# 412428728/ksched

Hardware: AMD Instinct MI355X
Metric: MCMF solve latency (ms) + arcs/s at 100k tasks x 10k machines, 1/2/4/8 GPUs (higher is better)
Workload: dtype int64; 1 GPU; config3: Quincy-shaped cell graph T=100000 M=10000 R=250 J=1000 (n=121252, m=531250), step = full device re-solve + device task->PU extraction (Solve() -> TaskMapping), one graph per GPU; tasks=100000, machines=10000, racks=250, jobs=1000, seed=3, n=121252, m=531250, parallelism=independent graphs x1

## Files before the change

### ksched_amd/csrc/ks_engine.hip

```cpp
#include <hip/hip_runtime.h>

#include <algorithm>
#include <chrono>
#include <cstdio>
#include <cstdlib>
#include <cstring>
#include <vector>

#include "ks_engine_impl.h"

namespace ks {
namespace {

__device__ __forceinline__ void seg_of(const long long* nd, int x, int& b0, int& b1) {
    const unsigned long long w = (unsigned long long)nd[ni(x) + ND_SEG];
    b0 = (int)(unsigned)(w & 0xffffffffULL);
    b1 = (int)(unsigned)(w >> 32);
}

__device__ __forceinline__ long long atom_add_ret(long long* p, long long v) {
    return __hip_atomic_fetch_add(p, v, __ATOMIC_RELAXED, __HIP_MEMORY_SCOPE_AGENT);
}
__device__ __forceinline__ long long atom_exch(long long* p, long long v) {
    return __hip_atomic_exchange(p, v, __ATOMIC_RELAXED, __HIP_MEMORY_SCOPE_AGENT);
// ... 727 lines not shown
    const unsigned long long sg = (unsigned long long)__shfl(f.seg, src);
    b0 = (int)(unsigned)(sg & 0xffffffffULL);
    en = (int)(unsigned)(sg >> 32);
}

#define KS_AFTER_LOADS(c0, c1, ...) asm volatile("" : "+v"(c0), "+v"(c1) : __VA_ARGS__)

template <int C, bool CP>
__device__ __forceinline__ void sweep_win(const DG& g, const Front& N, int w, unsigned long long mask,
                                          const WinFlag& f, const long long* __restrict__ P,
                                          long long* __restrict__ PN, long long eps, Pend& pd, int& out, Cnt& c) {
    constexpr int G = class_lanes(C);
    constexpr int PER = 64 / G;
    constexpr int WS = win_slots(C);
    const int base = g.obeg[C] + (w - g.wbeg[C]) * WS;
    const int k = lane_id() / G;
    while (mask) {
        unsigned long long mm = mask;
        for (int j = 0; j < k; ++j) mm &= mm - 1;
        const int v = mm ? base + __ffsll((long long)mm) - 1 : -1;
        long long e = 0, pv = 0;
        int b0 = 0, en = 0;
        window_node(f, v, base, e, pv, b0, en);
        if (v < 0) e = 0;
        sweep_group<G, CP>(g, N, v, e, pv, b0, en, PN, P, eps, pd, out, c);
        for (int j = 0; j < PER; ++j) mask &= mask - 1;
    }
}


template <bool CP>
__global__ __launch_bounds__(BLK) void k_sweep(DG g, int pos, int seq) {
    if (pos == 0 && blockIdx.x == 0 && threadIdx.x == 0) g.ctl->t_sw0 = __builtin_amdgcn_s_memrealtime();
    if (blockIdx.x == 0)
        for (int h = threadIdx.x; h < g.nheavy; h += BLK) g.sf[(seq + 2) % 3].hub[h] = 0;
    int c_done, c_act;
    auto ctl_words = [&]() {
        c_done = g.ctl->bf_done;
        c_act = pos == 0 ? g.ctl->apply_act : g.ctl->sweep_act[pos - 1];
    };
    const Front F = g.sf[seq % 3], N = g.sf[(seq + 1) % 3];
    const long long eps = g.ctl->eps;
    const long long* P = (pos & 1) ? g.p1 : g.p0;
    long long* PN = (pos & 1) ? g.p0 : g.p1;
    Pend pd{-1, 0};
    Cnt c;
    int out = 0;
    if ((int)blockIdx.x < g.nhitems) {
        const HItem it = g.hitems[blockIdx.x];
        const int fl = F.hub[it.hid];
        const long long px = P[ni(it.node)];
        const long long E = atom_load(&g.excess[it.node]);
        ctl_words();
        KS_AFTER_LOADS(c_done, c_act, "v"(fl), "v"(px), "v"(E));
        if (c_done && c_act && fl) {
            hub_chunk<CP>(g, F, N, it, px, E, P, PN, eps, pd, out, c);
        }
    } else if ((int)blockIdx.x >= g.nhitems + g.sw_clsb) {
        const int i = (int)blockIdx.x - g.nhitems - g.sw_clsb;
        if (i < g.ncls_c) {
            const int x = g.obeg[CCLS] + i;
            const int fl = F.flag[x];
            const long long e = atom_load(&g.excess[x]);
            const long long px = P[ni(x)];
            const long long sw = g.p0[ni(x) + ND_SEG];
            ctl_words();
            KS_AFTER_LOADS(c_done, c_act, "v"(fl), "v"(e), "v"(px), "v"(sw));
            const int b0 = (int)(unsigned)((unsigned long long)sw & 0xffffffffULL);
            const int en = (int)(unsigned)((unsigned long long)sw >> 32);
            __shared__ long long s_e;
            __shared__ int s_go;
            if (threadIdx.x == 0) {
                s_e = e;
                s_go = c_done && c_act && fl;
            }
            __syncthreads();
            if (s_go) {
                node_discharge_blk<CP>(g, F, N, x, s_e, px, b0, en, PN, P, eps, pd, out, c);
            }
        }
    } else {
        const int tw = g.sw_clsb * WPB;
        const int w0 = wave_index_in_grid(g.nhitems);
        WinFlag wf[WPW];
        int any_raw = 0;
#pragma unroll
        for (int j = 0; j < WPW; ++j) {
            const int w = w0 + j * tw;
            wf[j] = w < g.wbeg[CCLS] ? window_load<1>(g, F.flag, w, P) : WinFlag{-1, 0, 0, 0, 0};
            any_raw |= wf[j].raw;
        }
        ctl_words();
        KS_AFTER_LOADS(c_done, c_act, "v"(any_raw));
        const bool go = c_done && c_act;
        unsigned long long mk[WPW];
#pragma unroll
        for (int j = 0; j < WPW; ++j) mk[j] = window_take(g, F.flag, w0 + j * tw, wf[j], go);
#pragma unroll
        for (int j = 0; j < WPW; ++j) {
            if (!mk[j]) continue;
            const int w = w0 + j * tw;
            switch (class_of_window(g, w)) {
                case 0: sweep_win<0, CP>(g, N, w, mk[j], wf[j], P, PN, eps, pd, out, c); break;
                case 1: sweep_win<1, CP>(g, N, w, mk[j], wf[j], P, PN, eps, pd, out, c); break;
                case 2: sweep_win<2, CP>(g, N, w, mk[j], wf[j], P, PN, eps, pd, out, c); break;
                case 3: sweep_win<3, CP>(g, N, w, mk[j], wf[j], P, PN, eps, pd, out, c); break;
                default: sweep_win<4, CP>(g, N, w, mk[j], wf[j], P, PN, eps, pd, out, c); break;
            }
        }
    }
    if (__any(out) && lane_id() == 0) g.ctl->sweep_act[pos] = 1;
    flush_counters(g, c);
}

constexpr int PK_NB = 24;
constexpr long long PK_NONE = (1LL << PK_NB) - 1;
constexpr long long PK_BIAS = 1LL << 37;
__device__ __forceinline__ long long pk(long long d, long long v) {
    d = d < 1 - PK_BIAS ? 1 - PK_BIAS : (d > PK_BIAS - 1 ? PK_BIAS - 1 : d);
    return ((d + PK_BIAS) << PK_NB) | v;
}
__device__ __forceinline__ long long pk_d(long long key) { return (key >> PK_NB) - PK_BIAS; }
template <int PR>
__device__ __forceinline__ long long dkey(long long raw) { return PR == 2 ? pk_d(raw) : raw; }
template <int PR>
__device__ __forceinline__ bool dless(long long a, long long b) { return PR == 2 ? (a >> PK_NB) < (b >> PK_NB) : a < b; }

template <int PR>
__device__ __forceinline__ long long arc_len(long long pu, long long ca, long long pv, long long eps) {
    long long len = floordiv(pu - ca - pv, eps) + 1;
    if (!PR) len = len < 0 ? 0 : (len > LEN_CAP ? LEN_CAP : len);
    return len;
}

template <int PR>
__device__ __forceinline__ bool offer(const DG& g, const Front& nf, int u, long long cand, long long du,
                                      long long B, long long* hub_min, int& out) {
    if (cand >= B) return false;
    if (u >= g.hub_base) {
        const int h = u - g.hub_base;
        if (h < HUB_LDS) {
            __hip_atomic_fetch_min(&hub_min[h], cand, __ATOMIC_RELAXED, __HIP_MEMORY_SCOPE_WORKGROUP);
        } else if (dless<PR>(cand, atom_min_ret(&g.dist[ni(u)], cand))) {
            nf.hub[h] = 1;
            out = 1;
        }
        return false;
    }
    if (!dless<PR>(cand, du)) return false;
    atom_min(&g.dist[ni(u)], cand);
    return true;
}

template <int PR, bool CP>
__device__ __forceinline__ void expand_leaf(const DG& g, const Front& nf, int u, long long du, long long pu,
                                            int b0, int b1, long long eps, long long B, long long* hub_min, int& out,
                                            long long& lscan) {
    lscan += b1 - b0;
    unsigned live = 0;
    int hd[8];
    long long cb[8];
#pragma unroll
    for (int k = 0; k < 8; ++k) {
        hd[k] = 0;
        cb[k] = 0;
        if (b0 + k < b1) {
            const Pos q = PL<CP>::ld_nr(g, b0 + k);
            hd[k] = q.head;
            cb[k] = q.cost;
            if (q.ucap - q.rcap > 0) live |= 1u << k;
        }
    }
    for (int b = b1 - b0 > 8 ? b0 + 8 : b1; b < b1; ++b) {
        const Pos q = PL<CP>::ld_nr(g, b);
        if (q.ucap - q.rcap > 0) {
            const int u2 = q.head;
            long long cand = du + arc_len<PR>(g.p0[ni(u2)], q.cost, pu, eps);
            if (PR == 2) cand = pk(cand, b);
            if (offer<PR>(g, nf, u2, cand, u2 < g.hub_base ? g.dist[ni(u2)] : INF64, B, hub_min, out)) {
                nf.flag[u2] = 1;
                out = 1;
            }
        }
    }
    while (live) {
        const int k = __builtin_ctz(live);
        live &= live - 1;
        int u2 = 0;
        long long c2 = 0;
#pragma unroll
        for (int j = 0; j < 8; ++j)
            if (j == k) {
                u2 = hd[j];
                c2 = cb[j];
            }
        const long long pu2 = g.p0[ni(u2)];
        const long long du2 = u2 < g.hub_base ? g.dist[ni(u2)] : INF64;
        long long cand = du + arc_len<PR>(pu2, c2, pu, eps);
        if (PR == 2) cand = pk(cand, b0 + k);
        if (offer<PR>(g, nf, u2, cand, du2, B, hub_min, out)) {
            nf.flag[u2] = 1;
            out = 1;
        }
    }
}

template <int PR, bool CP>
__device__ __forceinline__ void relax_in(const DG& g, const Front& nf, int v, int a, long long dv, long long pv,
                                         long long eps, long long B, long long* hub_min, int& out, long long& lscan) {
    const Pos q = PL<CP>::ld_nr(g, a);
    const long long rin = q.ucap - q.rcap;
    const int u = rin > 0 ? q.head : 0;
    const long long ca = q.cost;
    const long long pu = g.p0[ni(u)];
    const long long du = u < g.hub_base ? g.dist[ni(u)] : INF64;
    const bool leaf = g.expand && u < g.obeg[2];
    int b0 = 0, b1 = 0;
    if (leaf) seg_of(g.p0, u, b0, b1);
    if (rin <= 0) return;
    const long long cand = dv + arc_len<PR>(pu, ca, pv, eps);
    if (!offer<PR>(g, nf, u, PR == 2 ? pk(cand, a) : cand, du, B, hub_min, out)) return;
    if (leaf) {
        expand_leaf<PR, CP>(g, nf, u, cand, pu, b0, b1, eps, B, hub_min, out, lscan);
    } else {
        nf.flag[u] = 1;
        out = 1;
    }
}

template <int G, int PR, bool CP>
__device__ __forceinline__ void bf_group_pre(const DG& g, const Front& nf, int v, long long dv, long long pv, int b0,
                                             int en, long long eps, long long B, long long* hub_min, int& out, long long& scans, long long& lscan) {
    const int lig = lane_id() & (G - 1);
    const bool act = v >= 0 && (PR || dv < INF64);
    if (!act) en = b0;
    const int iters = G < 64 ? 1 : (en - b0 + 63) / 64;
    for (int it = 0; it < iters; ++it) {
        const int a = b0 + it * G + lig;
        if (a < en) {
            relax_in<PR, CP>(g, nf, v, a, dkey<PR>(dv), pv, eps, B, hub_min, out, lscan);
            scans++;
        }
    }
}

template <int C, int PR, bool CP>
__device__ __forceinline__ void bf_win(const DG& g, const Front& N, int w, unsigned long long mask, const WinFlag& f,
                                       long long eps, long long B, long long* hub_min, int& out, long long& scans, long long& lscan) {
    constexpr int G = class_lanes(C);
    constexpr int PER = 64 / G;
    constexpr int WS = win_slots(C);
    const int base = g.obeg[C] + (w - g.wbeg[C]) * WS;
    const int k = lane_id() / G;
    while (mask) {
        unsigned long long mm = mask;
        for (int j = 0; j < k; ++j) mm &= mm - 1;
        const int v = mm ? base + __ffsll((long long)mm) - 1 : -1;
        long long d = INF64, pv = 0;
        int b0 = 0, en = 0;
        window_node(f, v, base, d, pv, b0, en);
        if (v < 0) d = INF64;
        bf_group_pre<G, PR, CP>(g, N, v, d, pv, b0, en, eps, B, hub_min, out, scans, lscan);
        for (int j = 0; j < PER; ++j) mask &= mask - 1;
    }
}

template <int PR, bool CP>
__device__ __forceinline__ void bf_chunk(const DG& g, const Front& N, const CItem& ci, long long eps,
                                         long long B, long long* hub_min, int& out, long long& scans, long long& lscan) {
    const long long dv = atom_load(&g.dist[ni(ci.node)]);
    if (!PR && dv >= INF64) return;
    const int a = ci.begin + lane_id();
    if (a < ci.end) {
        relax_in<PR, CP>(g, N, ci.node, a, dkey<PR>(dv), g.p0[ni(ci.node)], eps, B, hub_min, out, lscan);
        scans++;
    }
}

template <int G, int PR, bool CP>
__device__ __forceinline__ void bf_group(const DG& g, const Front& nf, int v, long long eps, long long B, long long* hub_min,
                                         int& out, long long& scans, long long& lscan) {
    const int lig = lane_id() & (G - 1);
    long long dv = INF64;
    if (v >= 0) dv = atom_load(&g.dist[ni(v)]);
    const bool act = v >= 0 && (PR || dv < INF64);
    long long pv = 0;
    int b0 = 0, en = 0;
    if (act) {
        pv = g.p0[ni(v)];
        seg_of(g.p0, v, b0, en);
    }
    const int iters = G < 64 ? 1 : (en - b0 + 63) / 64;
    for (int it = 0; it < iters; ++it) {
        const int a = b0 + it * G + lig;
        if (a < en) {
            relax_in<PR, CP>(g, nf, v, a, dkey<PR>(dv), pv, eps, B, hub_min, out, lscan);
            scans++;
        }
    }
}

template <int PR, bool CP>
__global__ __launch_bounds__(BLK) void k_bf_round(DG g, int seq, int dense_arg) {
    const unsigned long long t_entry = PR == 2 ? __builtin_amdgcn_s_memrealtime() : 0;
    const int dense = dense_arg >= 0 ? dense_arg : (seq == g.ctl->bf_seq0 ? 1 : 0);
    __shared__ long long hub_min[HUB_LDS];
    if (blockIdx.x == 0) {
        for (int h = threadIdx.x; h < g.nheavy; h += BLK) g.bf[(seq + 2) % 3].hub[h] = 0;
        if (threadIdx.x == 0) g.ctl->bfa[(seq + 2) % 3] = 0;
    }
    const Front F = g.bf[seq % 3], N = g.bf[(seq + 1) % 3];
    if (threadIdx.x < HUB_LDS) hub_min[threadIdx.x] = INF64;
    __syncthreads();
    int done = 0, any = 0;
    auto ctl_words = [&]() {
        done = g.ctl->bf_done;
        any = g.ctl->bfa[seq % 3];
    };
    const long long eps = g.ctl->eps;
    const long long B = (!PR && g.bound) ? atom_load(&g.ctl->bf_bound) : INF64;
    int out = 0;
    long long scans = 0, lscan = 0;
    const int nhb = g.nhitems * HSPLIT;
    if ((int)blockIdx.x < nhb) {
        const HItem it = g.hitems[blockIdx.x / HSPLIT];
        const int sub = (int)blockIdx.x % HSPLIT;
        const int fl = F.hub[it.hid];
        const long long dv = atom_load(&g.dist[ni(it.node)]);
        const long long pv = g.p0[ni(it.node)];
        ctl_words();
        KS_AFTER_LOADS(done, any, "v"(fl), "v"(dv), "v"(pv));
        if (!done && (dense || any) && (dense || fl)) {
            if (PR || dv < INF64) {
#pragma unroll
                for (int k = 0; k < BF_PER_T; ++k) {
                    const int a = it.begin + sub * (CHUNK / HSPLIT) + threadIdx.x * BF_PER_T + k;
                    if (a < it.end) {
                        relax_in<PR, CP>(g, N, it.node, a, dkey<PR>(dv), pv, eps, B, hub_min, out, lscan);
                        scans++;
                    }
                }
            }
        }
    } else if (dense) {
        const int w = wave_index_in_grid(nhb);
        ctl_words();
        if (done) {
        } else if (w < g.wbeg[CCLS]) {
            const Scan sc{F.flag, 1};
#define KS_BF_CALL(C) bf_group<G_, PR, CP>(g, N, v, eps, B, hub_min, out, scans, lscan)
            KS_BY_CLASS(w, sc, KS_BF_CALL)
#undef KS_BF_CALL
        } else if (w - g.wbeg[CCLS] < g.ncitems) {
            bf_chunk<PR, CP>(g, N, g.citems[w - g.wbeg[CCLS]], eps, B, hub_min, out, scans, lscan);
        }
    } else {
        const int tw = ((int)gridDim.x - nhb) * WPB;
        const int w0 = wave_index_in_grid(nhb);
        WinFlag wf[WPW];
        int any_raw = 0;
#pragma unroll
        for (int j = 0; j < WPW; ++j) {
            wf[j] = window_load<2>(g, F.flag, w0 + j * tw);
            any_raw |= wf[j].raw;
        }
        ctl_words();
        KS_AFTER_LOADS(done, any, "v"(any_raw));
        const bool go = !done && any;
        unsigned long long mk[WPW];
#pragma unroll
        for (int j = 0; j < WPW; ++j) {
            const int w = w0 + j * tw;
            mk[j] = window_take(g, F.flag, w, wf[j], go);
            if (go && w >= g.wbeg[CCLS] && w - g.wbeg[CCLS] < g.ncitems && lane_id() == 0) {
                const CItem ci = g.citems[w - g.wbeg[CCLS]];
                if (ci.lead) g.bf[(seq + 2) % 3].flag[ci.node] = 0;
            }
        }
#pragma unroll
        for (int j = 0; j < WPW; ++j) {
            if (!mk[j]) continue;
            const int w = w0 + j * tw;
            if (w >= g.wbeg[CCLS]) {
                bf_chunk<PR, CP>(g, N, g.citems[w - g.wbeg[CCLS]], eps, B, hub_min, out, scans, lscan);
                continue;
            }
            switch (class_of_window(g, w)) {
                case 0: bf_win<0, PR, CP>(g, N, w, mk[j], wf[j], eps, B, hub_min, out, scans, lscan); break;
                case 1: bf_win<1, PR, CP>(g, N, w, mk[j], wf[j], eps, B, hub_min, out, scans, lscan); break;
                case 2: bf_win<2, PR, CP>(g, N, w, mk[j], wf[j], eps, B, hub_min, out, scans, lscan); break;
                case 3: bf_win<3, PR, CP>(g, N, w, mk[j], wf[j], eps, B, hub_min, out, scans, lscan); break;
                default: bf_win<4, PR, CP>(g, N, w, mk[j], wf[j], eps, B, hub_min, out, scans, lscan); break;
            }
        }
    }
    __syncthreads();
    if (threadIdx.x < HUB_LDS && (int)threadIdx.x < g.nheavy) {
        const long long val = hub_min[threadIdx.x];
        if (val < INF64) {
            long long* dx = &g.dist[ni(g.hub_base + threadIdx.x)];
            if (dless<PR>(val, atom_load(dx)) && dless<PR>(val, atom_min_ret(dx, val))) {
                N.hub[threadIdx.x] = 1;
                out = 1;
            }
        }
    }
    if (__any(out) && lane_id() == 0) g.ctl->bfa[(seq + 1) % 3] = 1;
    if (blockIdx.x == 0 && threadIdx.x == 0) {
        if (PR == 2 && g.ctl->t_srch) {
            g.ctl->srch_ticks += t_entry - g.ctl->t_srch;
            g.ctl->t_srch = 0;
        }
        if (!done && (dense || any)) {
            atomicAdd(g.ctr + C_BFROUND, 1ULL);
            g.ctl->bf_count += 1;
        } else if (!done) {
            g.ctl->bf_done = 1;
        }
    }
    if (!PR && g.bound && blockIdx.x == 0 && threadIdx.x < WAVE && !done && (dense || any)) {
        const int nb = g.ctl->n_bx;
        if (nb > 0 && nb <= BX_CAP) {
            long long d = 0;
            if ((int)threadIdx.x < nb) d = atom_load(&g.dist[ni(g.bx[threadIdx.x])]);
            d = wave_max(d);
            if (threadIdx.x == 0 && d < INF64)
                __hip_atomic_fetch_min(&g.ctl->bf_bound, d, __ATOMIC_RELAXED, __HIP_MEMORY_SCOPE_AGENT);
        }
    }
    scans = wave_sum(scans);
    lscan = wave_sum(lscan);
    if (lane_id() == 0 && (scans | lscan)) {
        const int sh = ((blockIdx.x * WPB) + (threadIdx.x >> 6)) & (CTR_SHARDS - 1);
        if (scans) atomicAdd(g.ctr + sh * NCTR + C_GUSCAN, (unsigned long long)scans);
        if (lscan) atomicAdd(g.ctr + sh * NCTR + C_GULEAF, (unsigned long long)lscan);
    }
}

__device__ __forceinline__ void clear_fronts(const DG& g, const Front* fs) {
    for (long long i = blockIdx.x * (long long)BLK + threadIdx.x; i < g.hub_base; i += (long long)gridDim.x * BLK) {
        fs[0].flag[i] = 0;
        fs[1].flag[i] = 0;
        fs[2].flag[i] = 0;
    }
    if (blockIdx.x == 0)
        for (int h = threadIdx.x; h < g.nheavy; h += BLK) fs[0].hub[h] = fs[1].hub[h] = fs[2].hub[h] = 0;
}

__device__ __forceinline__ void bx_append(const DG& g, bool on, int v) {
    const unsigned long long m = __ballot(on);
    if (!m) return;
    int base = 0;
    if (lane_id() == 0) base = atomicAdd(&g.ctl->n_bx, (int)__popcll(m));
    base = __shfl(base, 0);
    if (on) {
        const int idx = base + (int)__popcll(m & ((1ULL << lane_id()) - 1));
        if (idx < BX_CAP) g.bx[idx] = v;
    }
}

__global__ void k_gu_init(DG g, int seq0, int list) {
    if (g.ctl->gu_pending) return;
    clear_fronts(g, g.bf);
    const Front F0 = g.bf[seq0 % 3];
    if (blockIdx.x == 0 && threadIdx.x == 0) {
        __hip_atomic_store(&g.ctl->bf_bound, INF64, __ATOMIC_RELAXED, __HIP_MEMORY_SCOPE_AGENT);
        g.ctl->gu_B = INF64;
        g.ctl->bf_done = 0;
        g.ctl->gu_L = 0;
        g.ctl->gu_X = -1;
        g.ctl->bf_r0 = g.ctl->bf_count;
        g.ctl->bf_seq0 = seq0;
        g.ctl->n_exc = 0;
        g.ctl->u_exc = 0;
        g.ctl->aug_reached = 0;
        g.ctl->aug_short = 0;
        for (int k = 0; k < 3; ++k) g.ctl->bfa[k] = k == seq0 % 3 ? 1 : 0;
    }
    for (long long v0 = blockIdx.x * (long long)BLK; v0 < g.hub_base; v0 += (long long)gridDim.x * BLK) {
        const long long v = v0 + threadIdx.x;
        long long e = 0;
        if (v < g.hub_base) {
            e = atom_load(&g.excess[v]);
            g.dist[ni(v)] = e < 0 ? 0 : INF64;
            if (e < 0) F0.flag[v] = 1;
        }
        if (list) bx_append(g, e > 0, (int)v);
    }
    if (blockIdx.x == 0)
        for (int h0 = 0; h0 < g.nheavy; h0 += BLK) {
            const int h = h0 + threadIdx.x;
            long long e = 0;
            if (h < g.nheavy) {
                drain_inbox(g, h);
                e = atom_load(&g.excess[g.hub_base + h]);
                g.dist[ni(g.hub_base + h)] = e < 0 ? 0 : INF64;
                if (e < 0) F0.hub[h] = 1;
            }
            if (list) bx_append(g, e > 0, g.hub_base + h);
        }
}

__global__ void k_pr_init(DG g, int seq0, int from_p) {
    clear_fronts(g, g.bf);
    if (blockIdx.x == 0 && threadIdx.x == 0) {
        g.ctl->bf_done = 0;
        g.ctl->bf_seq0 = seq0;
        for (int k = 0; k < 3; ++k) g.ctl->bfa[k] = 0;
    }
    for (long long v = blockIdx.x * (long long)BLK + threadIdx.x; v < g.n; v += (long long)gridDim.x * BLK)
        g.dist[ni(v)] = from_p == 2 ? ((PK_BIAS << PK_NB) | PK_NONE) : from_p ? g.p0[ni(v)] : 0;
}

__global__ void k_cycle_end(DG g, Ctl* host, int fwd) {
    static_assert(sizeof(Ctl) % 4 == 0, "Ctl is copied as words");
    const unsigned long long t = __builtin_amdgcn_s_memrealtime();
    if (threadIdx.x == 0) {
        if (!fwd) g.ctl->gu_pending = g.ctl->bf_done ? 0 : 1;
        g.ctl->t_end = t;
    }
    __syncthreads();
    const int* src = reinterpret_cast<const int*>(g.ctl);
    int* dst = reinterpret_cast<int*>(host);
    for (int i = threadIdx.x; i < (int)(sizeof(Ctl) / 4); i += blockDim.x)
        __hip_atomic_store(&dst[i], src[i], __ATOMIC_RELAXED, __HIP_MEMORY_SCOPE_SYSTEM);
    __syncthreads();
    if (threadIdx.x == 0) {
        if (!fwd) {
            g.ctl->n_exc = 0;
            g.ctl->u_exc = 0;
        }
        g.ctl->fs_moved_cyc = 0;
    }
    __threadfence_system();
}

constexpr int SET_FWD = 1;
constexpr int SET_CYC = 2;
__global__ void k_set_eps(DG g, long long eps, int flags) {
    g.ctl->eps = eps;
    if (flags & SET_FWD) {
        g.ctl->fs_pending = 0;
        g.ctl->fs_cnt[0] = g.ctl->fs_cnt[1] = g.ctl->fs_cnt[2] = 0;
        g.ctl->fs_completed = 0;
    }
    if (flags & SET_CYC) {
        g.ctl->cyc_done = 0;
        g.ctl->cyc_rej = 0;
    }
// ... 1214 lines not shown
        int nsearch, cap, used;
        int nb;
        unsigned long long srch_seen;
    } fin{};

    SolveRun(EngineImpl& s_, ks_result& res_, std::string& err_, bool warm)
        : s(s_), res(res_), err(err_), o(s_.opts), st(s_.stream), fb(s_.fb_active),
          use_warm((warm && s_.has_prev) || s_.fb_active) {}

    double wall_s() const {
        return std::chrono::duration<double>(std::chrono::steady_clock::now() - t_host0).count();
    }

    int run() {
        int rc = prepare();
        if (rc || nn == 0) return rc;
        plan();
        if ((rc = warm_start())) return rc;
        rc = s.cell_layout ? cell_solve() : phase_loop();
        if (rc || retry != RETRY_NONE) return rc;
        if (cycle_log)
            std::fprintf(stderr, "solve phases %d updates %llu (forward %llu) early phase ends %llu\n", phases,
                         (unsigned long long)gus, (unsigned long long)fwd_updates, (unsigned long long)early_exits);
        if (status == KS_E_INFEASIBLE && !s.cell_layout)
            err = "infeasible: some supply cannot reach a demand node (code " + std::to_string(s.h_ctl->infeasible) +
                  ", phase " + std::to_string(phases) + ", eps " + std::to_string(eps) + ", updates " +
                  std::to_string(gus) + ", sweeps " + std::to_string(sweep_launches) + ")";
        KS_CHECK(hipEventRecord(s.ev[5], st));
        if (status == KS_OK && (rc = certify())) return rc;
        return report();
    }

    int prepare() {
        s.solved = false;
        {
            const bool cells_now = want_cells(s);
            if (cells_now != s.cell_layout) {
                s.cell_layout = cells_now;
                s.csr_valid = false;
            }
        }
        res.warm_started = use_warm ? 1 : 0;
        res.rebuilt = s.csr_valid ? 0 : 1;
        res.recoveries = 0;
        res.cell_fallbacks = 0;
        res.cycles_cancelled = 0;
        res.fb_resets = 0;
        res.cycles_rejected = 0;
        KS_CHECK(hipEventRecord(s.ev[0], st));
        KS_CHECK(hipMemsetAsync(s.ctr.p, 0, CTR_SHARDS * NCTR * sizeof(unsigned long long), st));
        KS_CHECK(hipMemsetAsync(s.ctl.p, 0, sizeof(Ctl), st));
        std::memset(s.h_ctl, 0, sizeof(Ctl));
        if (!s.csr_valid) {
            if (int rc = rebuild()) return rc;
        } else if (!use_warm) {
            if (int rc = cold_reset(s, err)) return rc;
        }
        hi = s.hi();
        nn = s.nn;
        m2 = s.m2cap;
        mult = s.mult;
        ncells = (int)s.h_cells.size();
        res.n_nodes = s.nslots;
        res.n_arcs = s.h_sctl->live;
        if (nn == 0) {
            res.total_cost = 0;
            res.flow_value = 0;
            s.solved = true;
            s.has_prev = true;
            return KS_OK;
        }
        if (hi)
            hipLaunchKernelGGL(k_max_cost, dim3(grid_for(hi, 512)), dim3(BLK), 0, st, hi,
                               (const unsigned char*)s.a_alive.p, (const long long*)s.a_cost.p, &s.ctl.p->gu_L);
        const bool want_cp = !s.cell_layout && s.opts.compact_pos >= 0 && m2 > 0;
        if (want_cp) {
            KS_CHECK(s.cpos.ensure(m2));
            KS_CHECK(s.crev.ensure(m2));
            hipLaunchKernelGGL(k_pack_pos, dim3(grid_for(m2, 4096)), dim3(BLK), 0, st, (long long)m2,
                               (const Pos*)s.pos.p, s.cpos.p, s.crev.p, &s.ctl.p->cp_bad);
        }
        KS_CHECK(read_ctl());
        maxc = s.h_ctl->gu_L;
        cpv = want_cp && !s.h_ctl->cp_bad;
        cp_dirty = false;
        res.compact = cpv ? 1 : 0;
        KS_CHECK(hipMemsetAsync(&s.ctl.p->gu_L, 0, sizeof(long long), st));
        if (maxc > 0 && (double)maxc * (double)mult * 8.0 * (double)mult > 4.0e18) {
            err = "cost range too large for int64 scaled prices";
            return KS_E_RANGE;
        }
        KS_CHECK(hipEventRecord(s.ev[1], st));
        return KS_OK;
    }

    int rebuild() {
        const int64_t ncap_prev = s.ncap;
        const long long mult_prev = s.mult;
        const bool carry = use_warm && s.nn > 0;
        const int hi0 = s.hi();
        if (carry) {
            KS_CHECK(s.saved_flows.ensure(std::max(hi0, 1)));
            KS_CHECK(s.p_slot.ensure(std::max<int64_t>(ncap_prev, 1)));
            if (hi0)
                hipLaunchKernelGGL(k_save_flows, dim3(grid_for(hi0)), dim3(BLK), 0, st, hi0,
                                   (const unsigned char*)s.a_alive.p, (const int*)s.fwd.p, (const Pos*)s.pos.p,
                                   s.saved_flows.p);
            hipLaunchKernelGGL(k_save_prices, dim3(grid_for(ncap_prev)), dim3(BLK), 0, st, (int)ncap_prev,
                               (const int*)s.perm.p, (const long long*)s.nd.p, s.p_slot.p);
            if (fb && !s.fb_cells.empty()) {
                std::vector<long long> rng;
                const size_t kc = s.cell_off.size() >= 2 ? s.cell_off.size() - 1 : 1;
                for (int c : s.fb_cells) {
                    rng.push_back(kc > 1 ? s.cell_off[c] : 0);
                    rng.push_back(kc > 1 ? s.cell_off[c + 1] : ncap_prev);
                }
                KS_CHECK(s.fb_rng.ensure(rng.size()));
                KS_CHECK(hipMemcpyAsync(s.fb_rng.p, rng.data(), rng.size() * sizeof(long long), hipMemcpyHostToDevice,
                                        st));
                const int n = (int)std::max<int64_t>(hi0, ncap_prev);
                KS_CHECK(s.fb_cnt.ensure(1));
                KS_CHECK(hipMemsetAsync(s.fb_cnt.p, 0, sizeof(unsigned long long), st));
                hipLaunchKernelGGL(k_fb_reset, dim3(grid_for(std::max(n, 1))), dim3(BLK), 0, st, hi0, (int)ncap_prev,
                                   (int)(rng.size() / 2), (const long long*)s.fb_rng.p, (const int*)s.a_src.p,
                                   (const unsigned char*)s.a_alive.p, s.saved_flows.p, s.p_slot.p, s.fb_cnt.p);
                unsigned long long nres = 0;
                KS_CHECK(hipMemcpyAsync(&nres, s.fb_cnt.p, sizeof(nres), hipMemcpyDeviceToHost, st));
                KS_CHECK(hipStreamSynchronize(st));
                res.fb_resets = nres;
            }
        }
        int rc = build(s, err);
        if (rc) return rc;
        rc = cold_reset(s, err);
        if (rc) return rc;
        if (carry) {
            if (hi0)
                hipLaunchKernelGGL(k_restore_flows, dim3(grid_for(hi0)), dim3(BLK), 0, st, hi0,
                                   (const unsigned char*)s.a_alive.p, (const long long*)s.saved_flows.p,
                                   (const long long*)s.a_low.p, (const long long*)s.a_cap.p, (const int*)s.fwd.p,
                                   (const int*)s.a_src.p, (const int*)s.a_dst.p, (const int*)s.perm.p, s.pos.p,
                                   s.excess.p);
            hipLaunchKernelGGL(k_restore_prices, dim3(grid_for(s.ncap)), dim3(BLK), 0, st, (int)s.ncap,
                               (int)ncap_prev, mult_prev, s.mult, (const long long*)s.p_slot.p, (const int*)s.perm.p,
                               s.nd.p, (s.nd.p + 2));
        }
        return KS_OK;
    }

    void plan() {
        g = s.dg();
        g.cp = cpv ? s.cpos.p : nullptr;
        g.crev = cpv ? s.crev.p : nullptr;
        g.expand = o.two_hop < 0 ? 0 : 1;
        g.bound = o.bf_bound < 0 ? 0 : 1;
        g.fs_wide = std::max(2048, nn / 4);
        g.aug_k = o.tail_nodes > 0 ? std::min(AUG_KMAX, (int)o.tail_nodes) : 64;
        fgrid = s.window_grid();
        dgrid = s.dense_grid();
        sgrid = s.sparse_grid();
        wgrid = s.sweep_grid();
        ngrid = grid_for(nn, 2048);
        fsgrid = s.nhitems * HSPLIT + FS_LIST_BLOCKS;
        vgrid = grid_for(hi, 2048);
        use_fwd = o.fwd_nodes >= 0 && s.m2cap < FS_NONE;
        fwd_k = o.fwd_nodes > 0 ? (int)o.fwd_nodes : (nn < 32768 ? 32 : 64);
        use_pr = o.price_refine != 0;
        use_prc = use_pr && o.price_refine == 1 && !s.cell_layout && s.m2cap < PK_NONE;
        alpha = o.alpha >= 2 ? o.alpha : (!s.cell_layout && nn < 32768 && use_prc) ? 32 : 8;
        gi_base = o.gu_interval > 0 ? o.gu_interval : 24;
        gi_base = std::max(2, std::min(MAXB, gi_base)) & ~1;
        pr_cap = o.pr_rounds > 0 ? o.pr_rounds : 160;
        cycle_log = o.log_cycles != 0;
        nhit = s.nhitems;
        use_aug = o.walk_slack >= 0;
        aug_slack = o.walk_slack > 0 ? o.walk_slack : 4;
        walk_passes = o.walk_passes > 0 ? std::min(8, (int)o.walk_passes) : 1;
        kb_margin = o.bf_margin > 0 ? o.bf_margin : 6;
        kb_min = 8;
        prc_cap = (o.fault_inject & 32) ? 32 : 4096;
        cyc_lg = (o.fault_inject & 128) ? 5 : CYC_LOG;
        gi_tail = o.tail_sweeps > 0 ? std::max(2, std::min(MAXB, (int)o.tail_sweeps)) & ~1 : 4;
        phase_exit = o.phase_exit < 0 ? 0 : (o.phase_exit > 0 ? o.phase_exit : 256);
        phase_frac = o.phase_frac > 0 ? o.phase_frac : 128;
        eps = std::max<long long>(1, maxc * mult);
        {
            const long long D = o.final_div < 0 ? 0
                                : o.final_div > 0 ? o.final_div
                                : (s.cell_layout || nn < 32768) ? 20 : (use_prc ? 24 : 48);
            if (D > 0 && use_pr && maxc > 0) {
                long long e = std::max<long long>(1, (mult - 1) / D);
                if (s.cell_layout && (alpha & (alpha - 1)) == 0)
                    while (e & (e - 1)) e &= e - 1;
                const long long lo = std::max<long long>(1, eps / ((long long)alpha * alpha));
                while (e < lo && e <= (1LL << 58) / alpha) e *= alpha;
                eps = e * alpha;
                pr_div = D;
            }
        }
        eps_start = eps;
    }

    int warm_start() {
        if (!use_warm || fb) return KS_OK;
        if (o.warm_shift >= 0)
            hipLaunchKernelGGL(k_price_shift, dim3(grid_for(s.ncap, 2048)), dim3(BLK), 0, st, (int)s.ncap,
                               (const unsigned long long*)s.n_cshift.p, (const int*)s.perm.p, mult, s.nd.p);
        hipLaunchKernelGGL(k_fresh_prices, dim3(grid_for(s.ncap, 2048)), dim3(BLK), 0, st, (int)s.ncap,
                           (const unsigned char*)s.n_fresh.p, (const int*)s.perm.p, g);
        if (m2) hipLaunchKernelGGL(k_max_viol, dim3(grid_for(m2, 2048)), dim3(BLK), 0, st, g, (long long)m2);
        KS_CHECK(read_ctl());
        const long long viol = s.h_ctl->gu_L;
        constexpr long long kWarmUnits = 8;
        long long e0 = std::max<long long>(1, std::min<long long>({viol, kWarmUnits * mult, eps}));
        if (s.cell_layout && (alpha & (alpha - 1)) == 0)
            while (e0 & (e0 - 1)) e0 += e0 & -e0;
        warm_thr = e0;
        eps = e0 * alpha;
        eps_start = eps;
        KS_CHECK(hipMemsetAsync(&s.ctl.p->gu_L, 0, sizeof(long long), st));
        if (cycle_log) {
            std::vector<long long> h((size_t)4 * nn);
            KS_CHECK(hipMemcpyAsync(h.data(), s.nd.p, h.size() * sizeof(long long), hipMemcpyDeviceToHost, st));
            KS_CHECK(hipStreamSynchronize(st));
            long long lo = INF64, hi2 = -INF64;
            for (int v = 0; v < nn; ++v) {
                lo = std::min(lo, h[(size_t)4 * v]);
                hi2 = std::max(hi2, h[(size_t)4 * v]);
            }
            std::fprintf(stderr, "warm start: largest violation %.3f units, first phase at %.3f units, price span %.1f units\n",
                         (double)viol / mult, (double)e0 / mult, (double)(hi2 - lo) / mult);
        }
        return KS_OK;
    }

    hipError_t read_ctl() {
        hipError_t e = hipMemcpyAsync(s.h_ctl, s.ctl.p, sizeof(Ctl), hipMemcpyDeviceToHost, st);
        if (e != hipSuccess) return e;
        return hipStreamSynchronize(st);
    }
    hipError_t set_eps(long long e, int flags = 0) {
        hipLaunchKernelGGL(k_set_eps, dim3(1), dim3(1), 0, st, g, e, flags);
        return hipGetLastError();
    }
    void bf_round(int mode, bool dense) {
        const int grid = dense ? dgrid : sgrid;
        if (mode == 2) launch_bf_round<2>(cpv, grid, st, g, bseq, dense ? 1 : 0);
        else if (mode) launch_bf_round<1>(cpv, grid, st, g, bseq, dense ? 1 : 0);
        else launch_bf_round<0>(cpv, grid, st, g, bseq, dense ? 1 : 0);
        ++bseq;
        ++bf_launches;
    }
    void bf_rounds(int mode, int k, bool first_dense) {
        for (int r = 0; r < k; ++r) bf_round(mode, first_dense && r == 0);
    }
    void sync_pos() {
        if (!cp_dirty) return;
        hipLaunchKernelGGL(k_unpack_pos, dim3(grid_for(m2, 4096)), dim3(BLK), 0, st, (long long)m2,
                           (const CPos*)s.cpos.p, s.pos.p);
        cp_dirty = false;
    }
    int relaxations(unsigned long long* since) {
        std::vector<unsigned long long> hctr((size_t)CTR_SHARDS * NCTR);
        KS_CHECK(hipMemcpy(hctr.data(), s.ctr.p, hctr.size() * sizeof(unsigned long long), hipMemcpyDeviceToHost));
        unsigned long long gsc = 0;
        for (int i = 0; i < CTR_SHARDS; ++i) gsc += hctr[(size_t)i * NCTR + C_GUSCAN];
        *since = gsc - gu_prev;
        gu_prev = gsc;
        return KS_OK;
    }

    bool is_last(long long e) const { return e / alpha < 1 || e <= 1 || (use_pr && e * pr_div < mult); }

    int phase_loop() {
        do {
            eps = std::max<long long>(1, eps / alpha);
            ++phases;
            long long sat_thr = phases == 1 && use_warm && !fb
                                    ? warm_thr
                                    : ((pr_failed || fb || (use_warm && o.warm_start >= 2)) ? eps : 0LL);
            pr_failed = false;
            const bool last_phase = is_last(eps);
            const long long eps_next = std::max<long long>(1, eps / alpha);
            const bool before_last = !last_phase && !prc_tried && is_last(eps_next);
            const bool prc_now = use_prc && before_last;
            const long long eps_next2 = std::max<long long>(1, eps_next / alpha);
            const bool before_last2 = !last_phase && !before_last && is_last(eps_next2);
            const int walk_sl = (eps > 1 || (o.fault_inject & 1)) ? aug_slack : 1;
            int prc_early = 0;
            const bool may_early = use_prc && !prc_tried && before_last2 && !use_warm && !fb && eps <= 2 * mult;
            const int rc = run_phase(eps, sat_thr, !last_phase && !prc_now, walk_sl, may_early ? &prc_early : nullptr);
            if (rc == KS_E_INFEASIBLE) {
                status = rc;
                break;
            }
            if (rc) return rc;
            if (prc_now || prc_early) {
                prc_tried = true;
                int used = 0;
                const int pr = finish(&used, prc_early ? std::min(prc_cap, 1024) : prc_cap);
                if (pr < 0) return pr;
                if (pr == 1) {
                    eps = 1;
                    break;
                }
                pr_failed = true;
                continue;
// ... 689 lines not shown
```

Baseline: 15.53 million arcs/s.

## Drain newly improved mid-class nodes in-block via LDS queue during Bellman-Ford round

Adds a per-block shared-memory queue in the Bellman-Ford relaxation kernel. Nodes in a middle class range whose distance improves are queued, and the block drains them right away by scanning their arcs with 32-lane groups, instead of flagging them for the next global round. The drain skips entries whose distance has since changed. Two-hop expansion now defaults to mode 2, which enables the queue. The aim is to cut the number of global BF rounds and kernel launches, at the cost of extra LDS, atomics and a block-level sync.

```diff
diff --git a/ksched_amd/csrc/ks_engine.hip b/ksched_amd/csrc/ks_engine.hip
--- a/ksched_amd/csrc/ks_engine.hip
+++ b/ksched_amd/csrc/ks_engine.hip
@@ -903,8 +903,37 @@
     return true;
 }
 
+constexpr int TWO_HOP_DEFAULT = 2;
+constexpr int BF_DEPTH = 1;
+constexpr int BFQ_GROUP = 32;
+constexpr int BFQ_CAP = BLK / BFQ_GROUP;
+struct QEnt {
+    long long pu, d;
+    int b0, b1, u, pad;
+};
+struct BfQ {
+    QEnt* q;
+    int* n;
+    int cap;
+    int lo, hi;
+};
+__device__ __forceinline__ bool bf_enqueue(const BfQ& Q, int u, unsigned long long seg, long long d, long long pu) {
+    if (u < Q.lo || u >= Q.hi) return false;
+    const unsigned i = (unsigned)atomicAdd(Q.n, 1);
+    if (i >= (unsigned)Q.cap) return false;
+    QEnt e;
+    e.pu = pu;
+    e.d = d;
+    e.b0 = (int)(unsigned)(seg & 0xffffffffULL);
+    e.b1 = (int)(unsigned)(seg >> 32);
+    e.u = u;
+    e.pad = 0;
+    Q.q[i] = e;
+    return true;
+}
+
 template <int PR, bool CP>
-__device__ __forceinline__ void expand_leaf(const DG& g, const Front& nf, int u, long long du, long long pu,
+__device__ __forceinline__ void expand_leaf(const DG& g, const Front& nf, const BfQ& Q, int u, long long du, long long pu,
                                             int b0, int b1, long long eps, long long B, long long* hub_min, int& out,
                                             long long& lscan) {
     lscan += b1 - b0;
@@ -926,9 +955,11 @@
         const Pos q = PL<CP>::ld_nr(g, b);
         if (q.ucap - q.rcap > 0) {
             const int u2 = q.head;
-            long long cand = du + arc_len<PR>(g.p0[ni(u2)], q.cost, pu, eps);
+            const long long pu2 = g.p0[ni(u2)];
+            long long cand = du + arc_len<PR>(pu2, q.cost, pu, eps);
             if (PR == 2) cand = pk(cand, b);
-            if (offer<PR>(g, nf, u2, cand, u2 < g.hub_base ? g.dist[ni(u2)] : INF64, B, hub_min, out)) {
+            if (offer<PR>(g, nf, u2, cand, u2 < g.hub_base ? g.dist[ni(u2)] : INF64, B, hub_min, out) &&
+                !bf_enqueue(Q, u2, Q.cap ? (unsigned long long)g.p0[ni(u2) + ND_SEG] : 0ULL, dkey<PR>(cand), pu2)) {
                 nf.flag[u2] = 1;
                 out = 1;
             }
@@ -947,9 +978,10 @@
             }
         const long long pu2 = g.p0[ni(u2)];
         const long long du2 = u2 < g.hub_base ? g.dist[ni(u2)] : INF64;
+        const unsigned long long sg2 = Q.cap ? (unsigned long long)g.p0[ni(u2) + ND_SEG] : 0ULL;
         long long cand = du + arc_len<PR>(pu2, c2, pu, eps);
         if (PR == 2) cand = pk(cand, b0 + k);
-        if (offer<PR>(g, nf, u2, cand, du2, B, hub_min, out)) {
+        if (offer<PR>(g, nf, u2, cand, du2, B, hub_min, out) && !bf_enqueue(Q, u2, sg2, dkey<PR>(cand), pu2)) {
             nf.flag[u2] = 1;
             out = 1;
         }
@@ -957,30 +989,55 @@
 }
 
 template <int PR, bool CP>
-__device__ __forceinline__ void relax_in(const DG& g, const Front& nf, int v, int a, long long dv, long long pv,
-                                         long long eps, long long B, long long* hub_min, int& out, long long& lscan) {
-    const Pos q = PL<CP>::ld_nr(g, a);
+__device__ __forceinline__ void relax_pos(const DG& g, const Front& nf, const BfQ& Q, const Pos& q, int a, long long dv,
+                                          long long pv, long long eps, long long B, long long* hub_min, int& out,
+                                          long long& lscan) {
     const long long rin = q.ucap - q.rcap;
     const int u = rin > 0 ? q.head : 0;
     const long long ca = q.cost;
     const long long pu = g.p0[ni(u)];
     const long long du = u < g.hub_base ? g.dist[ni(u)] : INF64;
     const bool leaf = g.expand && u < g.obeg[2];
-    int b0 = 0, b1 = 0;
-    if (leaf) seg_of(g.p0, u, b0, b1);
+    unsigned long long sg = 0;
+    if (leaf || (u >= Q.lo && u < Q.hi)) sg = (unsigned long long)g.p0[ni(u) + ND_SEG];
     if (rin <= 0) return;
     const long long cand = dv + arc_len<PR>(pu, ca, pv, eps);
-    if (!offer<PR>(g, nf, u, PR == 2 ? pk(cand, a) : cand, du, B, hub_min, out)) return;
+    const long long key = PR == 2 ? pk(cand, a) : cand;
+    if (!offer<PR>(g, nf, u, key, du, B, hub_min, out)) return;
     if (leaf) {
-        expand_leaf<PR, CP>(g, nf, u, cand, pu, b0, b1, eps, B, hub_min, out, lscan);
-    } else {
+        const int b0 = (int)(unsigned)(sg & 0xffffffffULL), b1 = (int)(unsigned)(sg >> 32);
+        expand_leaf<PR, CP>(g, nf, Q, u, cand, pu, b0, b1, eps, B, hub_min, out, lscan);
+    } else if (!bf_enqueue(Q, u, sg, dkey<PR>(key), pu)) {
         nf.flag[u] = 1;
         out = 1;
     }
 }
 
+template <int PR, bool CP>
+__device__ __forceinline__ void relax_in(const DG& g, const Front& nf, const BfQ& Q, int v, int a, long long dv, long long pv,
+                                         long long eps, long long B, long long* hub_min, int& out, long long& lscan) {
+    relax_pos<PR, CP>(g, nf, Q, PL<CP>::ld_nr(g, a), a, dv, pv, eps, B, hub_min, out, lscan);
+}
+
+template <int PR, bool CP>
+__device__ __forceinline__ void bf_drain(const DG& g, const Front& nf, const QEnt* q, int n, const BfQ& Qn, long long eps,
+                                         long long B, long long* hub_min, int& out, long long& scans, long long& lscan) {
+    constexpr int QG = BFQ_GROUP;
+    const int lig = threadIdx.x & (QG - 1);
+    for (int i = threadIdx.x / QG; i < n; i += BLK / QG) {
+        const QEnt e = q[i];
+        const long long cur = atom_load(&g.dist[ni(e.u)]);
+        for (int a = e.b0 + lig; a < e.b1; a += QG) {
+            Pos p = PL<CP>::ld_nr(g, a);
+            if (dkey<PR>(cur) != e.d) p.rcap = p.ucap;
+            relax_pos<PR, CP>(g, nf, Qn, p, a, e.d, e.pu, eps, B, hub_min, out, lscan);
+            scans++;
+        }
+    }
+}
+
 template <int G, int PR, bool CP>
-__device__ __forceinline__ void bf_group_pre(const DG& g, const Front& nf, int v, long long dv, long long pv, int b0,
+__device__ __forceinline__ void bf_group_pre(const DG& g, const Front& nf, const BfQ& Q, int v, long long dv, long long pv, int b0,
                                              int en, long long eps, long long B, long long* hub_min, int& out, long long& scans, long long& lscan) {
     const int lig = lane_id() & (G - 1);
     const bool act = v >= 0 && (PR || dv < INF64);
@@ -989,14 +1046,14 @@
     for (int it = 0; it < iters; ++it) {
         const int a = b0 + it * G + lig;
         if (a < en) {
-            relax_in<PR, CP>(g, nf, v, a, dkey<PR>(dv), pv, eps, B, hub_min, out, lscan);
+            relax_in<PR, CP>(g, nf, Q, v, a, dkey<PR>(dv), pv, eps, B, hub_min, out, lscan);
             scans++;
         }
     }
 }
 
 template <int C, int PR, bool CP>
-__device__ __forceinline__ void bf_win(const DG& g, const Front& N, int w, unsigned long long mask, const WinFlag& f,
+__device__ __forceinline__ void bf_win(const DG& g, const Front& N, const BfQ& Q, int w, unsigned long long mask, const WinFlag& f,
                                        long long eps, long long B, long long* hub_min, int& out, long long& scans, long long& lscan) {
     constexpr int G = class_lanes(C);
     constexpr int PER = 64 / G;
@@ -1011,25 +1068,25 @@
         int b0 = 0, en = 0;
         window_node(f, v, base, d, pv, b0, en);
         if (v < 0) d = INF64;
-        bf_group_pre<G, PR, CP>(g, N, v, d, pv, b0, en, eps, B, hub_min, out, scans, lscan);
+        bf_group_pre<G, PR, CP>(g, N, Q, v, d, pv, b0, en, eps, B, hub_min, out, scans, lscan);
         for (int j = 0; j < PER; ++j) mask &= mask - 1;
     }
 }
 
 template <int PR, bool CP>
-__device__ __forceinline__ void bf_chunk(const DG& g, const Front& N, const CItem& ci, long long eps,
+__device__ __forceinline__ void bf_chunk(const DG& g, const Front& N, const BfQ& Q, const CItem& ci, long long eps,
                                          long long B, long long* hub_min, int& out, long long& scans, long long& lscan) {
     const long long dv = atom_load(&g.dist[ni(ci.node)]);
     if (!PR && dv >= INF64) return;
     const int a = ci.begin + lane_id();
     if (a < ci.end) {
-        relax_in<PR, CP>(g, N, ci.node, a, dkey<PR>(dv), g.p0[ni(ci.node)], eps, B, hub_min, out, lscan);
+        relax_in<PR, CP>(g, N, Q, ci.node, a, dkey<PR>(dv), g.p0[ni(ci.node)], eps, B, hub_min, out, lscan);
         scans++;
     }
 }
 
 template <int G, int PR, bool CP>
-__device__ __forceinline__ void bf_group(const DG& g, const Front& nf, int v, long long eps, long long B, long long* hub_min,
+__device__ __forceinline__ void bf_group(const DG& g, const Front& nf, const BfQ& Q, int v, long long eps, long long B, long long* hub_min,
                                          int& out, long long& scans, long long& lscan) {
     const int lig = lane_id() & (G - 1);
     long long dv = INF64;
@@ -1045,7 +1102,7 @@
     for (int it = 0; it < iters; ++it) {
         const int a = b0 + it * G + lig;
         if (a < en) {
-            relax_in<PR, CP>(g, nf, v, a, dkey<PR>(dv), pv, eps, B, hub_min, out, lscan);
+            relax_in<PR, CP>(g, nf, Q, v, a, dkey<PR>(dv), pv, eps, B, hub_min, out, lscan);
             scans++;
         }
     }
@@ -1056,12 +1113,18 @@
     const unsigned long long t_entry = PR == 2 ? __builtin_amdgcn_s_memrealtime() : 0;
     const int dense = dense_arg >= 0 ? dense_arg : (seq == g.ctl->bf_seq0 ? 1 : 0);
     __shared__ long long hub_min[HUB_LDS];
+    __shared__ QEnt bfq[BF_DEPTH][BFQ_CAP];
+    __shared__ int bfq_n[BF_DEPTH];
     if (blockIdx.x == 0) {
         for (int h = threadIdx.x; h < g.nheavy; h += BLK) g.bf[(seq + 2) % 3].hub[h] = 0;
         if (threadIdx.x == 0) g.ctl->bfa[(seq + 2) % 3] = 0;
     }
     const Front F = g.bf[seq % 3], N = g.bf[(seq + 1) % 3];
     if (threadIdx.x < HUB_LDS) hub_min[threadIdx.x] = INF64;
+    if (threadIdx.x < BF_DEPTH) bfq_n[threadIdx.x] = 0;
+    const int qcap = g.expand < 2 ? 0 : (g.expand == 2 ? BFQ_CAP : 2);
+    const int qlo = qcap ? g.obeg[2] : 0, qhi = qcap ? g.obeg[CCLS] : 0;
+    const BfQ Q{bfq[0], &bfq_n[0], qcap, qlo, qhi};
     __syncthreads();
     int done = 0, any = 0;
     auto ctl_words = [&]() {
@@ -1087,7 +1150,7 @@
                 for (int k = 0; k < BF_PER_T; ++k) {
                     const int a = it.begin + sub * (CHUNK / HSPLIT) + threadIdx.x * BF_PER_T + k;
                     if (a < it.end) {
-                        relax_in<PR, CP>(g, N, it.node, a, dkey<PR>(dv), pv, eps, B, hub_min, out, lscan);
+                        relax_in<PR, CP>(g, N, Q, it.node, a, dkey<PR>(dv), pv, eps, B, hub_min, out, lscan);
                         scans++;
                     }
                 }
@@ -1099,11 +1162,11 @@
         if (done) {
         } else if (w < g.wbeg[CCLS]) {
             const Scan sc{F.flag, 1};
-#define KS_BF_CALL(C) bf_group<G_, PR, CP>(g, N, v, eps, B, hub_min, out, scans, lscan)
+#define KS_BF_CALL(C) bf_group<G_, PR, CP>(g, N, Q, v, eps, B, hub_min, out, scans, lscan)
             KS_BY_CLASS(w, sc, KS_BF_CALL)
 #undef KS_BF_CALL
         } else if (w - g.wbeg[CCLS] < g.ncitems) {
-            bf_chunk<PR, CP>(g, N, g.citems[w - g.wbeg[CCLS]], eps, B, hub_min, out, scans, lscan);
+            bf_chunk<PR, CP>(g, N, Q, g.citems[w - g.wbeg[CCLS]], eps, B, hub_min, out, scans, lscan);
         }
     } else {
         const int tw = ((int)gridDim.x - nhb) * WPB;
@@ -1133,19 +1196,29 @@
             if (!mk[j]) continue;
             const int w = w0 + j * tw;
             if (w >= g.wbeg[CCLS]) {
-                bf_chunk<PR, CP>(g, N, g.citems[w - g.wbeg[CCLS]], eps, B, hub_min, out, scans, lscan);
+                bf_chunk<PR, CP>(g, N, Q, g.citems[w - g.wbeg[CCLS]], eps, B, hub_min, out, scans, lscan);
                 continue;
             }
             switch (class_of_window(g, w)) {
-                case 0: bf_win<0, PR, CP>(g, N, w, mk[j], wf[j], eps, B, hub_min, out, scans, lscan); break;
-                case 1: bf_win<1, PR, CP>(g, N, w, mk[j], wf[j], eps, B, hub_min, out, scans, lscan); break;
-                case 2: bf_win<2, PR, CP>(g, N, w, mk[j], wf[j], eps, B, hub_min, out, scans, lscan); break;
-                case 3: bf_win<3, PR, CP>(g, N, w, mk[j], wf[j], eps, B, hub_min, out, scans, lscan); break;
-                default: bf_win<4, PR, CP>(g, N, w, mk[j], wf[j], eps, B, hub_min, out, scans, lscan); break;
+                case 0: bf_win<0, PR, CP>(g, N, Q, w, mk[j], wf[j], eps, B, hub_min, out, scans, lscan); break;
+                case 1: bf_win<1, PR, CP>(g, N, Q, w, mk[j], wf[j], eps, B, hub_min, out, scans, lscan); break;
+                case 2: bf_win<2, PR, CP>(g, N, Q, w, mk[j], wf[j], eps, B, hub_min, out, scans, lscan); break;
+                case 3: bf_win<3, PR, CP>(g, N, Q, w, mk[j], wf[j], eps, B, hub_min, out, scans, lscan); break;
+                default: bf_win<4, PR, CP>(g, N, Q, w, mk[j], wf[j], eps, B, hub_min, out, scans, lscan); break;
             }
         }
     }
     __syncthreads();
+    if (bfq_n[0]) {
+#pragma unroll
+        for (int l = 0; l < BF_DEPTH; ++l) {
+            const int qn = min(bfq_n[l], qcap);
+            const BfQ Qn{bfq[l + 1 < BF_DEPTH ? l + 1 : 0], &bfq_n[l + 1 < BF_DEPTH ? l + 1 : 0],
+                         l + 1 < BF_DEPTH ? qcap : 0, l + 1 < BF_DEPTH ? qlo : 0, l + 1 < BF_DEPTH ? qhi : 0};
+            bf_drain<PR, CP>(g, N, bfq[l], qn, Qn, eps, B, hub_min, out, scans, lscan);
+            __syncthreads();
+        }
+    }
     if (threadIdx.x < HUB_LDS && (int)threadIdx.x < g.nheavy) {
         const long long val = hub_min[threadIdx.x];
         if (val < INF64) {
@@ -2666,7 +2739,10 @@
         g = s.dg();
         g.cp = cpv ? s.cpos.p : nullptr;
         g.crev = cpv ? s.crev.p : nullptr;
-        g.expand = o.two_hop < 0 ? 0 : 1;
+        {
+            const int hops = o.two_hop < 0 ? 0 : (o.two_hop == 0 ? TWO_HOP_DEFAULT : std::min(2, (int)o.two_hop));
+            g.expand = (hops == 2 && (o.fault_inject & 512)) ? 3 : hops;
+        }
         g.bound = o.bf_bound < 0 ? 0 : 1;
         g.fs_wide = std::max(2048, nn / 4);
         g.aug_k = o.tail_nodes > 0 ? std::min(AUG_KMAX, (int)o.tail_nodes) : 64;
```

Result: faster. 15.99 million arcs/s (median of 6 runs) (+2.9%).
